# finsberg/fenicsx-beat

Hardware: AMD Instinct MI355X
Metric: node_updates_per_sec (higher is better)
Workload: dtype f64

## Files before the change

### fenicsx-beat_amd/beat/_engine.py

```python

from __future__ import annotations

import ctypes as C
import os
from dataclasses import dataclass
from typing import Any

import numpy as np

from . import _hip


@dataclass
class Slab:

    nz_global: int
    rank: int = 0
    world: int = 1
    weights: Any = None

    def __post_init__(self):
        if self.world > self.nz_global:
            raise ValueError(f"{self.world} ranks for only {self.nz_global} z-planes")
        if self.weights is not None and self.world > 1:
# ... 345 lines not shown
        if isinstance(order, str):
            if order != "auto":
                raise ValueError(f"guess order must be an integer 0..4 or 'auto', got {order!r}")
            order = -1
        self.flush_pending()
        _hip.check(self.lib.beat_pde_set_guess_order(self.handle, int(order)))
        self.guess_order = int(order)

    def set_single_reduction(self, on) -> None:
        _hip.check(self.lib.beat_pde_set_single_reduction(self.handle, -1 if on is None else int(bool(on))))

    def set_small(self, enable: bool) -> None:
        _hip.check(self.lib.beat_pde_set_small_grid_solve(self.handle, int(bool(enable))))

    def small_active(self) -> bool:
        return bool(self.lib.beat_pde_small_grid_solve_active(self.handle))

    RR_ROUTE_KEYS = ("available", "ry", "pd", "by_rows_mask", "nsegx", "nrb", "zc", "nchunks", "total_blocks", "guess_ry")

    def rr_route(self) -> dict:
        out = (C.c_int * len(self.RR_ROUTE_KEYS))()
        _hip.check(self.lib.beat_pde_rr_route(self.handle, out))
        return {k: int(v) for k, v in zip(self.RR_ROUTE_KEYS, out)}

    def guess_traffic(self) -> dict:
        out = (C.c_int * 4)()
        _hip.check(self.lib.beat_pde_guess_traffic(self.handle, out))
        return {"reads": int(out[0]), "writes": int(out[1]), "order": int(out[2]), "pending": bool(out[3])}

    def guess_reset(self) -> None:
        self.flush_pending()
        _hip.check(self.lib.beat_pde_guess_reset(self.handle))

    def flush_pending(self) -> None:
        if self.open_x is not None:
            self.solve_finish()
        if self.pending is not None:
            x, ring_base, _ = self.pending
            self.pending = None
            self.flushes = getattr(self, "flushes", 0) + 1
            _hip.check(self.lib.beat_pde_x_flush(self.handle, C.c_void_p(self.st_ptr_for_flush), x.ptr, self.ring[0].ptr,
                                                 self.fld, ring_base, 0))

    def flush_pending_events(self, field, maps, t0: float, t1: float) -> bool:
        if self.open_x is not None:
            self.solve_finish()
# ... 485 lines not shown
```

### fenicsx-beat_amd/beat/_hip.py

```python

from __future__ import annotations

import ctypes as C
import os
from pathlib import Path

_HERE = Path(__file__).resolve().parent
_LIB_PATH = Path(os.environ.get("BEAT_HIP_LIBRARY", _HERE / "lib" / "libbeat_hip.so"))

MODEL_SIMPLE_ODE = 0
MODEL_FHN_DEMO = 1
MODEL_FHN_README = 2
MODEL_TP06_GRL1 = 3
MODEL_TORORD_DYNCL_GRL1 = 4
MODEL_TORORD_LAND_GRL1 = 5
(MATH_EXP, MATH_EXP_INT, MATH_LOG, MATH_LOG_INT, MATH_RCP, MATH_RSQRT, MATH_TP06_RCP2, MATH_TP06_RCP3, MATH_TP06_RCP4,
 MATH_TORORD_RCP2, MATH_TORORD_RCP3, MATH_TORORD_RCP4, MATH_TP06_PHI_SMALL, MATH_TP06_PHI7, MATH_TORORD_PHI_SMALL,
 MATH_TORORD_PHI7, MATH_TP06_GRL1, MATH_TP06_ADVANCE, MATH_TP06_GATE, MATH_TORORD_ADVANCE, MATH_TORORD_GATE,
 MATH_TORORD_GATE_B) = range(22)
MATH_IN = (1, 1, 1, 1, 1, 1, 2, 3, 4, 2, 3, 4, 1, 1, 1, 1, 4, 4, 4, 4, 4, 4)
MATH_OUT = (1, 1, 1, 1, 1, 1, 2, 3, 4, 2, 3, 4, 1, 1, 1, 1, 1, 1, 1, 1, 1, 1)
MAX_STIM = 8
MAX_CLASSES = 32
MAX_LEADS = 16
# ... 80 lines not shown
    "beat_pde_set_timestep": (_int, [_vp, _dbl, _dbl, _dbl]),
    "beat_pde_apply": (_int, [_vp, _int, _vp, _vp]),
    "beat_pde_rhs": (_int, [_vp, _vp, C.POINTER(_vp), C.POINTER(_dbl), _int, _vp, _vp, _vp, _vp]),
    "beat_pde_cg_begin": (_int, [_vp, _vp, _dbl, _dbl, _int]),
    "beat_pde_spmv_dot": (_int, [_vp, _vp, _vp, _vp]),
    "beat_pde_spmv_dot_part": (_int, [_vp, _vp, _vp, _vp, _int]),
    "beat_pde_cg_update": (_int, [_vp, _vp, _vp, _vp, _vp, _vp]),
    "beat_pde_cg_next": (_int, [_vp, _vp, _vp, _vp]),
    "beat_pde_ring_size": (_int, []),
    "beat_pde_cg_update_r": (_int, [_vp, _vp, _vp, _vp, _int]),
    "beat_pde_cg_next_oop": (_int, [_vp, _vp, _vp, _vp, _vp]),
    "beat_pde_x_flush": (_int, [_vp, _vp, _vp, _vp, _i64, _int, _int]),
    "beat_pde_set_small_grid_solve": (_int, [_vp, _int]),
    "beat_pde_small_grid_solve_active": (_int, [_vp]),
    "beat_split_steps": (_int, [_vp, _int, _vp, _i64, _i64, _vp, _int, _int, _vp, _int, _vp, _vp, _vp, _vp, _int, _dbl, _dbl,
                                _int, _vp, _vp, _int, _vp, _vp]),
    "beat_split_steps_big": (_int, [_vp, _int, _vp, _i64, _i64, _vp, _int, _int, _vp, _vp, _int, _vp, _vp, _vp, _vp, _int, _dbl, _dbl, _int, _int,
                             C.POINTER(KspInfo), C.POINTER(_int), C.POINTER(C.c_float)]),
    "beat_pde_set_guess_order": (_int, [_vp, _int]),
    "beat_pde_set_single_reduction": (_int, [_vp, _int]),
    "beat_pde_fused_dist_pass": (_int, [_vp]),
    "beat_pde_tile_route": (_int, [_vp]),
    "beat_pde_rr_route": (_int, [_vp, C.POINTER(_int)]),
    "beat_pde_guess_reset": (_int, [_vp]),
    "beat_pde_guess_pending": (_int, [_vp]),
    "beat_pde_guess_history": (_int, [_vp, _vp, _vp, _vp]),
    "beat_pde_guess_traffic": (_int, [_vp, C.POINTER(_int)]),
    "beat_pde_set_preconditioner": (_int, [_vp, _int, _vp]),
    "beat_pde_pc_num_passes": (_int, [_vp]),
    "beat_pde_pc_pass": (_int, [_vp, _int, _vp, _vp, _vp, _vp, _vp]),
    "beat_pde_cg_first_z": (_int, [_vp, _vp, _vp, _vp]),
    "beat_pde_cg_next_z": (_int, [_vp, _vp, _vp, _vp]),
    "beat_pde_work_fields": (_int, [_vp]),
    "beat_pde_field_stride": (_i64, [_vp]),
    "beat_pde_solve": (
        _int,
        [_vp, _vp, C.POINTER(_vp), C.POINTER(_dbl), _int, _vp, _vp, _dbl, _dbl, _int, C.POINTER(KspInfo)],
    ),
    "beat_pde_solve_begin": (_int, [_vp, _vp, C.POINTER(_vp), C.POINTER(_dbl), _int, _vp, _vp, _dbl, _dbl, _int]),
    "beat_pde_solve_end": (_int, [_vp, C.POINTER(KspInfo), C.POINTER(_int)]),
    "beat_pde_solve_is_open": (_int, [_vp]),
    "beat_pde_solve_can_open": (_int, [_vp]),
    "beat_pde_solve_ex": (
        _int,
        [_vp, _vp, C.POINTER(_vp), C.POINTER(_dbl), _int, _vp, _vp, _dbl, _dbl, _int, _int, C.POINTER(KspInfo), C.POINTER(_int)],
    ),
# ... 93 lines not shown
```

### fenicsx-beat_amd/csrc/beat_pde_rr.hip

```cpp
#include "beat_pde_internal.h"

#include <algorithm>
#include <cmath>
#include <cstddef>
#include <cstdlib>

namespace {
using namespace beat_pde_detail;

constexpr int SEG = 62;

struct Coef {
  double c[15];
};

struct RGeom {
  int nx, ny, nz;
  int64_t plane;
  int ry;
  int nsegx, nrb, nchunks, zc;
  int total_waves, total_blocks;
  int z_lo_phys, z_hi_phys;
  int z_lo, z_hi;
  int part_off;
// ... 84 lines not shown
#define BEAT_RR_ALIGN_RHS 0
#endif
constexpr bool rr_aligned_mode(int mode) {
  return BEAT_RR_ALIGN == 1 && BEAT_RR_BUF != 0 && (mode == 0 || mode == 1 || mode == 3 || mode == 4 || (mode == 2 && BEAT_RR_ALIGN_RHS == 1));
}

__device__ __forceinline__ int axis_type3(int i, int n, int lo_phys, int hi_phys) {
  if (n == 1 && lo_phys && hi_phys) return 1;
  if (i == 0 && lo_phys) return 0;
  if (i == n - 1 && hi_phys) return 2;
  return 1;
}

__device__ __forceinline__ int xcd_block(int b, int total) {
  const int per = (total + 7) >> 3;
  return (b & 7) * per + (b >> 3);
}

#ifndef BEAT_RR_WAVES_RHS
#define BEAT_RR_WAVES_RHS 3
#endif
#ifndef BEAT_RR_WAVES_IT
#define BEAT_RR_WAVES_IT 1
#endif
template <int MODE, int RY, int PD, bool GUESS = false, bool PRED = false>
__global__ __launch_bounds__(BEAT_BLOCK, (GUESS && RY == 2 && PD == 1) ? BEAT_RR_WAVES_RHS : ((MODE == RR_PDOT || MODE == RR_RUPD) && PD == 1 ? BEAT_RR_WAVES_IT : 1)) void rr_kernel(RGeom g, RArgs a, const double* __restrict__ X,
                                                        const double* __restrict__ X2, double* __restrict__ Y,
                                                        double* __restrict__ Y2) {
  constexpr int NR = RY + 2;
  constexpr int NE = GUESS ? NR : 1;
  constexpr bool FORM = MODE == RR_PDOT || MODE == RR_UDOT || MODE == RR_PRUPD;
  constexpr bool OLD = MODE == RR_PDOT || MODE == RR_PRUPD;
  constexpr bool RAW = MODE == RR_UDOT || MODE == RR_PRUPD;
  constexpr int NW = RAW ? RY : 1;
  constexpr bool BUF = BEAT_RR_BUF == 1 || (BEAT_RR_BUF == 2 && (MODE != RR_RHS || BEAT_RR_ALIGN_RHS == 1));
  constexpr bool ALIGNED = rr_aligned_mode(MODE);
  static_assert(!ALIGNED || BUF, "aligned segments come with the raw-buffer loads");
  constexpr int SEGW = ALIGNED ? 64 : SEG;
  static_assert(!GUESS || MODE == RR_RHS, "the initial guess enters the right-hand side only");
  static_assert(!PRED || MODE == RR_PDOT, "the predicted-stop sums come with PDOT only");
  __shared__ double red[4];
  __shared__ double s_dinv[32];
  __shared__ double s_tab[27 * TABW];
  __shared__ double s_tab2[MODE == RR_RHS ? 27 * TABW : 1];
  __shared__ double s_taba[GUESS ? 27 * TABW : 1];
  __shared__ double s_rc[PRED ? 4 * 2 * RY * 64 : 1];
// ... 358 lines not shown
  if (MODE == RR_PDOT && !PRED) {
    const double s0 = beat_block_sum(acc0, red);
    if (threadIdx.x == 0) a.partials[g.part_off + blockIdx.x] = s0;
  } else if (MODE == RR_RUPD) {
    const double s0 = beat_block_sum(acc0, red);
    const double s1 = beat_block_sum(acc1, red);
    if (threadIdx.x == 0) {
      a.partials[g.part_off + blockIdx.x] = s0;
      a.partials[BEAT_MAX_PARTIALS + g.part_off + blockIdx.x] = s1;
    }
  } else if (MODE == RR_PRUPD) {
  } else {
    const double s0 = beat_block_sum(acc0, red);
    const double s1 = beat_block_sum(acc1, red);
    const double s2 = beat_block_sum(acc2, red);
    if (threadIdx.x == 0) {
      a.partials[g.part_off + blockIdx.x] = s0;
      a.partials[BEAT_MAX_PARTIALS + g.part_off + blockIdx.x] = s1;
      a.partials[2 * BEAT_MAX_PARTIALS + g.part_off + blockIdx.x] = s2;
    }
  }
}

__global__ void rr_next_kernel(double* st) {
  if (st[STOP] != 0.0) return;
  st[BETA] = st[RZN] / st[RZ];
  st[RZ] = st[RZN];
  st[RR] = st[RRN];
  st[ITERS] += 1.0;
  const double tr = st[RTOL] * st[RTOL] * st[BB];
  if (st[RR] <= st[TOL2]) {
    st[STOP] = 1.0;
    st[REASON] = st[RR] <= tr ? 2.0 : 3.0;
  } else if (st[ITERS] >= st[MAXIT]) {
    st[STOP] = 1.0;
    st[REASON] = -3.0;
  }
}

__global__ void rr_merged_next_kernel(double* st, double* alphas, int slot) {
  if (st[STOP] != 0.0) return;
  const double g = st[RZN], d = st[PQ], rr = st[RRN];
  st[RR] = rr;
  const double tr = st[RTOL] * st[RTOL] * st[BB];
  if (rr <= st[TOL2]) {
    st[STOP] = 1.0;
// ... 37 lines not shown
    const int v = e ? std::atoi(e) : 1;
    return (v >= 1 && v <= 3) ? v : 1;
  }();
  return pd;
}

int rr_guess_rows() {
  static const int rows = [] {
    const char* e = std::getenv("BEAT_RR_GUESS_RY");
    const int v = e ? std::atoi(e) : 2;
    return v == 4 ? 4 : 2;
  }();
  return rows;
}

int rr_by_rows_mask() {
  static const int mask = [] {
    const char* e = std::getenv("BEAT_RR_BY_ROWS");
    return e ? std::atoi(e) : 0;
  }();
  return mask;
}

RGeom make_geom(const beat_pde* pde, int z_lo, int z_hi, int part_off, int rows = 0, int mode = -1) {
  const Geom& f = pde->g;
  RGeom g{};
  const int64_t nodes = (int64_t)f.nx * f.ny * f.nz;
  const int RY = g.ry = rows ? rows : rr_rows(nodes);
  g.nx = f.nx;
  g.ny = f.ny;
  g.nz = f.nz;
  g.plane = f.plane;
  g.z_lo_phys = f.z_lo_phys;
  g.z_hi_phys = f.z_hi_phys;
  g.z_lo = z_lo;
  g.z_hi = z_hi;
  g.part_off = part_off;
  g.ghost_lo_tz = pde->ghost_lo_tz;
  g.ghost_hi_tz = pde->ghost_hi_tz;
  const int segw = (mode >= 0 && rr_aligned_mode(mode)) ? 64 : SEG;
  g.nsegx = (f.nx + segw - 1) / segw;
  g.nrb = (f.ny + RY - 1) / RY;
  const int nzr = std::max(0, z_hi - z_lo);
  g.nrg = (mode >= 0 && ((rr_by_rows_mask() >> mode) & 1)) ? (g.nrb + 3) / 4 : 0;
  const int64_t per_layer = g.nrg > 0 ? (int64_t)g.nsegx * g.nrg : ((int64_t)g.nsegx * g.nrb + 3) / 4;
  const int target = rr_target_blocks(nodes);
  int nchunks = (int)std::max<int64_t>(1, (target + per_layer - 1) / per_layer);
  nchunks = std::max(1, std::min(nchunks, nzr));
  g.zc = std::max(1, (nzr + nchunks - 1) / nchunks);
  g.nchunks = (nzr + g.zc - 1) / g.zc;
  while ((int64_t)g.nsegx * g.nrb * g.nchunks > (int64_t)2 * BEAT_MAX_PARTIALS && g.nchunks > 1) {
    g.zc *= 2;
    g.nchunks = (nzr + g.zc - 1) / g.zc;
  }
  g.total_waves = g.nsegx * g.nrb * g.nchunks;
  g.total_blocks = (g.total_waves + 3) / 4;
  if (g.nrg > 0) {
    g.total_blocks = g.nsegx * g.nrg * g.nchunks;
    g.total_waves = g.total_blocks * 4;
  }
  return g;
}

// ... 14 lines not shown
  a.dinv = pde->d_dinv();
  a.ci = interior_row(pde->h_A);
  a.dinv_i = pde->h_dinv[13];
  a.partials = pde->ctx->d_partials;
  a.st = dev_st;
  return a;
}

template <int MODE, bool GUESS = false, bool PRED = false>
void launch_rr(const beat_pde* pde, const RGeom& g, const RArgs& a) {
  if (g.total_blocks <= 0) return;
  const dim3 grid((unsigned)grid_blocks(g)), block(BEAT_BLOCK);
  hipStream_t s = pde->ctx->stream;
#define BEAT_RR_LAUNCH(RYV, PDV) \
  BEAT_KERNEL((rr_kernel<MODE, RYV, PDV, GUESS, PRED>), grid, block, 0, s, g, a, a.x, GUESS ? a.e : a.x2, a.y, a.y2)
  const int pd = rr_prefetch();
  if (g.ry == 2) {
    if (pd == 2) BEAT_RR_LAUNCH(2, 2); else if (pd == 3) BEAT_RR_LAUNCH(2, 3); else BEAT_RR_LAUNCH(2, 1);
  } else {
    if (pd == 2) BEAT_RR_LAUNCH(4, 2); else if (pd == 3) BEAT_RR_LAUNCH(4, 3); else BEAT_RR_LAUNCH(4, 1);
  }
#undef BEAT_RR_LAUNCH
}
}

bool beat_rr_available(const beat_pde* pde) {
  if (pde->var || pde->pc_ncoef != 1) return false;
  if (const char* e = std::getenv("BEAT_RR")) {
    if (e[0] == '0') return false;
  }
  const RGeom g = make_geom(pde);
  const RGeom gb = make_geom(pde, 0, 1, 0);
  return (int64_t)grid_blocks(g) + 2 * grid_blocks(gb) <= BEAT_MAX_PARTIALS;
}

extern "C" int beat_pde_rr_route(const beat_pde* pde, int* host_out) {
  BEAT_REQUIRE(pde != nullptr && host_out != nullptr, "null argument");
  const RGeom g = make_geom(pde, 0, pde->g.nz, 0, 0, RR_PDOT);
  host_out[0] = beat_rr_available(pde) ? 1 : 0;
  host_out[1] = g.ry;
  host_out[2] = rr_prefetch();
  host_out[3] = rr_by_rows_mask();
  host_out[4] = g.nsegx;
  host_out[5] = g.nrb;
  host_out[6] = g.zc;
  host_out[7] = g.nchunks;
  host_out[8] = g.total_blocks;
  host_out[9] = rr_guess_rows();
  return BEAT_OK;
}

int beat_rr_rhs(beat_pde* pde, const double* dev_v_prev, const double* const* host_dev_stim_w, const double* host_stim_amp,
                int n_stim, double* dev_x, double* dev_r, double* dev_st, int part, const PcgStart* start) {
  BEAT_REQUIRE(start == nullptr || part < 0, "only a right-hand side in one part starts the solve");
  const GuessTerms& gt = pde->guess.cur;
  const bool guess = gt.d != nullptr && gt.use_e;
  const int rows = guess ? rr_guess_rows() : 0;
  RArgs a{};
  a.x = dev_v_prev;
  a.y = dev_r;
  a.y2 = (dev_x == dev_v_prev) ? nullptr : dev_x;
  a.tab = pde->d_tab(2);
  a.tab2 = pde->d_tab(3);
  a.dinv = pde->d_dinv();
  a.ci = interior_row(pde->h_mass);
  a.ci2 = interior_row(pde->h_stiff);
  a.dinv_i = pde->h_dinv[13];
  a.cm = pde->C_m;
  a.omt_dt = (1.0 - pde->theta) * pde->dt;
  a.dt = pde->dt;
  beat_fill_stimuli(a, host_dev_stim_w, host_stim_amp, n_stim);
// ... 2 lines not shown
  if (guess) {
    a.tab = pde->d_tab(1);
    a.ci = interior_row(pde->h_B);
    a.e = gt.e;
    a.taba = pde->d_tab(0);
    a.cia = interior_row(pde->h_A);
  }
  auto launch = [&](int z_lo, int z_hi, int part_off) {
    const RGeom g = make_geom(pde, z_lo, z_hi, part_off, rows, RR_RHS);
    if (guess)
      launch_rr<RR_RHS, true>(pde, g, a);
    else
      launch_rr<RR_RHS>(pde, g, a);
    return blocks_written(g);
  };
  int count = 0;
  if (int rc = beat_launch_parts(pde, PASS_RR_RHS, part, launch, &count)) return rc;
  return part == 0 ? BEAT_OK : beat_pde_launch_reduce(pde, count, 3, dev_st, nullptr, ScalarStep::begin(dev_st, start));
}

double beat_rr_predict_bound(const beat_pde* pde) {
  const Geom& f = pde->g;
  int depth = 0;
  auto chain = [&](const RGeom& g) {
    const int per_thread = (grid_blocks(g) + BEAT_BLOCK - 1) / BEAT_BLOCK;
    depth = std::max(depth, g.zc * g.ry + 8 + per_thread + 8);
  };
  chain(make_geom(pde, 0, f.nz, 0, 0, RR_RHS));
  chain(make_geom(pde, 0, f.nz, 0, 2, RR_RHS));
  chain(make_geom(pde, 0, f.nz, 0, 4, RR_RHS));
  chain(make_geom(pde, 0, f.nz, 0, 0, RR_PDOT));
  chain(make_geom(pde, 0, f.nz, 0, 0, RR_RUPD));
  return 4.0 * (2.0 * depth + 8.0) * std::ldexp(1.0, -53);
}

int beat_rr_pdot_part(beat_pde* pde, double* dev_st, const double* dev_r, const double* dev_p_old, double* dev_p_new,
                      int part, int slot) {
  const Geom& f = pde->g;
  const bool pred = slot >= 0 && pde->predict_stop && f.z_lo_phys && f.z_hi_phys;
  if (pred && pde->predict_c <= 0.0) pde->predict_c = beat_rr_predict_bound(pde);
  RArgs a = rr_operator_args(pde, dev_st);
  a.x = dev_r;
  a.x2 = dev_p_old;
  a.y = dev_p_new;
  auto launch = [&](int z_lo, int z_hi, int part_off) {
    const RGeom g = make_geom(pde, z_lo, z_hi, part_off, 0, RR_PDOT);
    if (pred)
      launch_rr<RR_PDOT, false, true>(pde, g, a);
    else
      launch_rr<RR_PDOT>(pde, g, a);
    return blocks_written(g);
  };
  int count = 0;
  if (int rc = beat_launch_parts(pde, PASS_RR_PDOT, part, launch, &count)) return rc;
  if (part == 0) return BEAT_OK;
  if (pred) {
    static_assert(RQ == PQS + 1 && QQ == PQS + 2, "the three sums are reduced into one run of slots");
    ScalarStep predict{ScalarStep::PREDICT, dev_st};
    predict.alpha_slot = pde->d_alphas + slot;
    predict.bound_c = pde->predict_c;
    return beat_pde_launch_reduce(pde, count, 3, dev_st + PQS, dev_st, predict);
  }
  return beat_pde_launch_reduce(pde, count, 1, dev_st + PQ, dev_st);
}

int beat_rr_pdot(beat_pde* pde, double* dev_st, const double* dev_r, const double* dev_p_old, double* dev_p_new, int slot) {
  if (int rc = beat_rr_pdot_part(pde, dev_st, dev_r, dev_p_old, dev_p_new, 0, slot)) return rc;
  return beat_rr_pdot_part(pde, dev_st, dev_r, dev_p_old, dev_p_new, 1, slot);
}

int beat_rr_rupd(beat_pde* pde, double* dev_st, const double* dev_r, double* dev_r_new, const double* dev_p, int slot,
                 bool roll) {
  const RGeom g = make_geom(pde, 0, pde->g.nz, 0, 0, RR_RUPD);
  RArgs a = rr_operator_args(pde, dev_st);
  a.x = dev_p;
  a.x2 = dev_r;
  a.y = dev_r_new;
  a.alphas = pde->d_alphas;
  a.slot = slot;
  launch_rr<RR_RUPD>(pde, g, a);
  BEAT_LAUNCH_CHECK();
  return beat_pde_launch_reduce(pde, grid_blocks(g), 2, dev_st + RZN, dev_st, ScalarStep::after_update(dev_st, roll));
}

int beat_rr_udot_part(beat_pde* pde, double* dev_st, const double* dev_r, int part) {
  static_assert(RZN == PQ + 1 && RRN == PQ + 2, "the three sums travel as one all-reduce of dev_st[PQ..RRN]");
  RArgs a = rr_operator_args(pde, dev_st);
  a.x = dev_r;
  a.x2 = dev_r;
  auto launch = [&](int z_lo, int z_hi, int part_off) {
    const RGeom g = make_geom(pde, z_lo, z_hi, part_off, 0, RR_UDOT);
    launch_rr<RR_UDOT>(pde, g, a);
    return blocks_written(g);
  };
  int count = 0;
  if (int rc = beat_launch_parts(pde, PASS_RR_UDOT, part, launch, &count)) return rc;
  return part == 0 ? BEAT_OK : beat_pde_launch_reduce(pde, count, 3, dev_st + PQ, dev_st);
}

int beat_rr_merged_next(beat_pde* pde, double* dev_st, int slot) {
  BEAT_KERNEL(rr_merged_next_kernel, dim3(1), dim3(1), 0, pde->ctx->stream, dev_st, pde->d_alphas, slot);
  BEAT_LAUNCH_CHECK();
  return BEAT_OK;
// ... 21 lines not shown
```

### fenicsx-beat_amd/csrc/beat_probe.hip

```cpp
#include "beat_common.h"
#include "beat_math_probe.h"

namespace {

typedef double v2d __attribute__((ext_vector_type(2)));
typedef int v4i __attribute__((ext_vector_type(4)));

template <int POL>
__device__ __forceinline__ v2d ld16(const v2d* base, int64_t i) {
  if constexpr (POL & 4) {
    const int64_t blk = i >> 26;
    const __amdgpu_buffer_rsrc_t r = __builtin_amdgcn_make_buffer_rsrc((void*)(base + (blk << 26)), 0, 0x7ffffff0, 0x00020000);
    const v4i v = __builtin_amdgcn_raw_buffer_load_b128(r, (int)((i - (blk << 26)) * 16), 0, (POL & 1) ? 2 : 0);
    return __builtin_bit_cast(v2d, v);
  } else if constexpr (POL & 1) {
    return __builtin_nontemporal_load(base + i);
  } else {
    return base[i];
  }
}
template <int POL>
__device__ __forceinline__ void st16(v2d* base, int64_t i, v2d v) {
  if constexpr (POL & 4) {
    const int64_t blk = i >> 26;
// ... 121 lines not shown
    for (int r = 0; r < NR; ++r) nxt[r] = src[(int64_t)zn * plane + off[r]];
    double hnxt = 0.0;
    if (halo) {
      const __amdgpu_buffer_rsrc_t rs = __builtin_amdgcn_make_buffer_rsrc((void*)(src + (int64_t)zn * plane), 0, (int)(plane * 8), 0x00020000);
      typedef int v2i __attribute__((ext_vector_type(2)));
      const v2i hv = __builtin_amdgcn_raw_buffer_load_b64(rs, (int)hoff, 0, 0);
      hnxt = __hiloint2double(hv.y, hv.x);
    }
    if (out) {
#pragma unroll
      for (int j = 0; j < RY; ++j) {
        const int gy = rb * RY + j;
        if (gy < ny) dst[(int64_t)z * plane + (int64_t)gy * nx + gx] = cur[j] + cur[j + 1] + cur[j + 2] + (lane == 0 ? hcur : 0.0);
      }
    }
    hsum += hcur;
#pragma unroll
    for (int r = 0; r < NR; ++r) cur[r] = nxt[r];
    hcur = hnxt;
  }
  if (hsum == 1.2345e300) dst[0] = hsum;
}

int launch_march(beat_ctx* ctx, double* dev, int64_t n, int nx, int ry, int segw, int shift, int blocks, int halo) {
  BEAT_REQUIRE(nx >= 64 && (segw == 62 || segw == 64) && (shift == 0 || shift == -1) && (ry == 2 || ry == 4), "bad march probe arguments");
  const int64_t per_field = n / 2;
  const int nz = (int)(per_field / ((int64_t)nx * nx));
  BEAT_REQUIRE(nz >= 1 && (int64_t)nz * nx * nx == per_field, "the buffer holds two fields of nx x nx x nz doubles");
  const int nseg = (nx + segw - 1) / segw, nrb = (nx + ry - 1) / ry;
  const int64_t per_layer = ((int64_t)nseg * nrb + 3) / 4;
  int nchunks = (int)std::max<int64_t>(1, ((blocks > 0 ? blocks : 4096) + per_layer - 1) / per_layer);
  nchunks = std::min(nchunks, nz);
  const int zc = (nz + nchunks - 1) / nchunks;
  nchunks = (nz + zc - 1) / zc;
  const int total_waves = nseg * nrb * nchunks;
  const unsigned grid = (unsigned)((total_waves + 3) / 4);
  if (ry == 4)
    BEAT_KERNEL((march_kernel<4>), dim3(grid), dim3(BEAT_BLOCK), 0, ctx->stream, (const double*)dev, dev + per_field, nx, nx, nz, segw, shift, zc, total_waves, halo);
  else
    BEAT_KERNEL((march_kernel<2>), dim3(grid), dim3(BEAT_BLOCK), 0, ctx->stream, (const double*)dev, dev + per_field, nx, nx, nz, segw, shift, zc, total_waves, halo);
  BEAT_LAUNCH_CHECK();
  return BEAT_OK;
}

__global__ __launch_bounds__(BEAT_BLOCK) void math_probe_kernel(int fn, const double* __restrict__ in, int64_t ld, double* __restrict__ out,
                                                                int64_t n) {
  __shared__ double etab[BEAT_EXP_TAB], etabi[BEAT_EXP_TAB];
  __shared__ LogEntry ltab[128];
  static_assert(BEAT_EXP_TAB == BEAT_BLOCK, "one table entry per thread");
  etab[threadIdx.x] = beat_exp_tab_entry<false>(kExp2Tab[threadIdx.x], (int)threadIdx.x);
  etabi[threadIdx.x] = beat_exp_tab_entry<true>(kExp2Tab[threadIdx.x], (int)threadIdx.x);
  if (threadIdx.x < 128) ltab[threadIdx.x] = kLogTab[threadIdx.x];
  __syncthreads();
  FastMath fm{etab, ltab};
  FastMathT<true> fmi{etabi, ltab};
  beat_fm_pin(fm);
  beat_fm_pin(fmi);
  const int64_t i = (int64_t)blockIdx.x * BEAT_BLOCK + threadIdx.x;
  if (i >= n) return;
  double a[4], o[4];
// ... 52 lines not shown
```

### include/beat_hip.h

```cpp
#ifndef BEAT_HIP_H
#define BEAT_HIP_H

#include <stddef.h>
#include <stdint.h>

#ifdef __cplusplus
extern "C" {
#endif

#define BEAT_OK 0
#define BEAT_EINVAL -1
#define BEAT_EHIP -2
#define BEAT_ENOTCONV -3
#define BEAT_ENOMEM -4

#define BEAT_ABI_VERSION 1

#define BEAT_MODEL_SIMPLE_ODE 0
#define BEAT_MODEL_FHN_DEMO 1
#define BEAT_MODEL_FHN_README 2
#define BEAT_MODEL_TP06_GRL1 3

#define BEAT_MODEL_TORORD_DYNCL_GRL1 4
#define BEAT_MODEL_TORORD_LAND_GRL1 5
// ... 99 lines not shown
int beat_pde_cg_next(beat_pde* pde, double* dev_st, const double* dev_r, double* dev_p);

int beat_pde_ring_size(void);
int beat_pde_cg_update_r(beat_pde* pde, double* dev_st, double* dev_r, const double* dev_q, int slot);
int beat_pde_cg_next_oop(beat_pde* pde, double* dev_st, const double* dev_r, const double* dev_p_cur,
                         double* dev_p_next);
int beat_pde_x_flush(beat_pde* pde, const double* dev_st, double* dev_x, const double* dev_ring0,
                     int64_t field_stride, int ring_base, int only_if_full);

int beat_pde_set_preconditioner(beat_pde* pde, int ncoef, const double* host_coef);
int beat_pde_pc_num_passes(beat_pde* pde);
int beat_pde_pc_pass(beat_pde* pde, int j, const double* dev_r, double* dev_z, double* dev_q,
                     double* dev_st, double* dev_red);
int beat_pde_cg_first_z(beat_pde* pde, double* dev_st, const double* dev_z, double* dev_p);
int beat_pde_cg_next_z(beat_pde* pde, double* dev_st, const double* dev_z, double* dev_p);

int beat_pde_work_fields(beat_pde* pde);
int64_t beat_pde_field_stride(const beat_pde* pde);
int beat_pde_set_guess_order(beat_pde* pde, int order);
int beat_pde_set_single_reduction(beat_pde* pde, int on);
int beat_pde_fused_dist_pass(const beat_pde* pde);
int beat_pde_tile_route(const beat_pde* pde);
int beat_pde_rr_route(const beat_pde* pde, int* host_out);
int beat_pde_guess_reset(beat_pde* pde);
int beat_pde_guess_pending(const beat_pde* pde);
int beat_pde_guess_history(const beat_pde* pde, double** dev_d, double** dev_e, int* count);
int beat_pde_guess_traffic(const beat_pde* pde, int* host_out);

int beat_pde_set_small_grid_solve(beat_pde* pde, int enable);
int beat_pde_small_grid_solve_active(const beat_pde* pde);

#define BEAT_MAX_BATCH 1024
int beat_split_steps(beat_ctx* ctx, int model_id, double* dev_states, int64_t n, int64_t ld,
                     const double* host_params, int num_params, int v_index, beat_pde* pde, int n_steps,
                     const double* host_t0, const double* host_dt, const double* const* host_dev_stim_w, const double* host_stim_amp, int n_stim,
                     double rtol, double atol, int max_it, const int64_t* host_probe_idx, const double* host_probe_w,
                     int n_probe, double* dev_probe_out, beat_ksp_info* host_info);
int beat_split_steps_big(beat_ctx* ctx, int model_id, double* dev_states, int64_t n, int64_t ld, const double* host_params,
                         int num_params, int v_index, beat_pde* pde, double* dev_work, int n_steps, const double* host_t0,
                         const double* host_dt, const double* const* host_dev_stim_w, const double* host_stim_amp, int n_stim,
                         double rtol, double atol, int max_it, int pending_in, beat_ksp_info* host_info, int* host_pending,
                         float* host_ode_ms);

int beat_pde_solve_begin(beat_pde* pde, const double* dev_v_prev, const double* const* host_dev_stim_w,
                         const double* host_stim_amp, int n_stim, double* dev_x, double* dev_work, double rtol, double atol, int max_it);
int beat_pde_solve_end(beat_pde* pde, beat_ksp_info* info, int* host_pending);
// ... 92 lines not shown
```

Baseline: 11.29 billion.

## Process two x-nodes per lane in the CG stencil pdot and residual-update kernels

Adds an rr2_kernel variant in which each lane handles two adjacent x nodes using 128-bit buffer loads and stores, with segments widened to 128 nodes. It is used by default for the PDOT and RUPD iteration passes when nx is even and the aligned prefetch route is active. The aim is to halve the number of load/store instructions and give each lane more independent arithmetic, at the cost of higher register pressure and a 16-byte alignment requirement on the vectors. A matching march probe kernel and a query for the element count are also added.

```diff
diff --git a/fenicsx-beat_amd/beat/_engine.py b/fenicsx-beat_amd/beat/_engine.py
--- a/fenicsx-beat_amd/beat/_engine.py
+++ b/fenicsx-beat_amd/beat/_engine.py
@@ -391,6 +391,11 @@
         out = (C.c_int * len(self.RR_ROUTE_KEYS))()
         _hip.check(self.lib.beat_pde_rr_route(self.handle, out))
         return {k: int(v) for k, v in zip(self.RR_ROUTE_KEYS, out)}
+
+    def rr_elems(self) -> int:
+        out = (C.c_int * 1)()
+        _hip.check(self.lib.beat_pde_rr_elems(self.handle, out))
+        return int(out[0])
 
     def guess_traffic(self) -> dict:
         out = (C.c_int * 4)()
diff --git a/fenicsx-beat_amd/beat/_hip.py b/fenicsx-beat_amd/beat/_hip.py
--- a/fenicsx-beat_amd/beat/_hip.py
+++ b/fenicsx-beat_amd/beat/_hip.py
@@ -126,6 +126,7 @@
     "beat_pde_fused_dist_pass": (_int, [_vp]),
     "beat_pde_tile_route": (_int, [_vp]),
     "beat_pde_rr_route": (_int, [_vp, C.POINTER(_int)]),
+    "beat_pde_rr_elems": (_int, [_vp, C.POINTER(_int)]),
     "beat_pde_guess_reset": (_int, [_vp]),
     "beat_pde_guess_pending": (_int, [_vp]),
     "beat_pde_guess_history": (_int, [_vp, _vp, _vp, _vp]),
diff --git a/fenicsx-beat_amd/csrc/beat_pde_rr.hip b/fenicsx-beat_amd/csrc/beat_pde_rr.hip
--- a/fenicsx-beat_amd/csrc/beat_pde_rr.hip
+++ b/fenicsx-beat_amd/csrc/beat_pde_rr.hip
@@ -130,6 +130,9 @@
 #endif
 #ifndef BEAT_RR_WAVES_IT
 #define BEAT_RR_WAVES_IT 1
+#endif
+#ifndef BEAT_RR_ELEMS_DEFAULT
+#define BEAT_RR_ELEMS_DEFAULT 2
 #endif
 template <int MODE, int RY, int PD, bool GUESS = false, bool PRED = false>
 __global__ __launch_bounds__(BEAT_BLOCK, (GUESS && RY == 2 && PD == 1) ? BEAT_RR_WAVES_RHS : ((MODE == RR_PDOT || MODE == RR_RUPD) && PD == 1 ? BEAT_RR_WAVES_IT : 1)) void rr_kernel(RGeom g, RArgs a, const double* __restrict__ X,
@@ -534,6 +537,252 @@
   }
 }
 
+typedef double rr_v2d __attribute__((ext_vector_type(2)));
+typedef int rr_v4i __attribute__((ext_vector_type(4)));
+constexpr int SEG2 = 128;
+__device__ __forceinline__ rr_v2d rr_buf_load2(const double* base, unsigned bytes, unsigned off) {
+  const __amdgpu_buffer_rsrc_t r = __builtin_amdgcn_make_buffer_rsrc((void*)base, 0, (int)bytes, 0x00020000);
+  return __builtin_bit_cast(rr_v2d, __builtin_amdgcn_raw_buffer_load_b128(r, (int)off, 0, (BEAT_RR_NT & 1) ? 2 : 0));
+}
+__device__ __forceinline__ void rr_store2(double* p, rr_v2d v) {
+#if BEAT_RR_NT & 2
+  __builtin_nontemporal_store(v, (rr_v2d*)p);
+#else
+  *(rr_v2d*)p = v;
+#endif
+}
+
+template <int MODE, int RY, bool PRED = false>
+__global__ __launch_bounds__(BEAT_BLOCK, BEAT_RR_WAVES_IT) void rr2_kernel(RGeom g, RArgs a, const double* __restrict__ X,
+                                                                             const double* __restrict__ X2, double* __restrict__ Y) {
+  static_assert(MODE == RR_PDOT || MODE == RR_RUPD, "two nodes per lane: the iteration's two passes only");
+  static_assert(!PRED || MODE == RR_PDOT, "the predicted-stop sums come with PDOT only");
+  static_assert(rr_aligned_mode(MODE), "the aligned raw-buffer form");
+  constexpr int NR = RY + 2;
+  constexpr bool FORM = MODE == RR_PDOT;
+  __shared__ double red[4];
+  __shared__ double s_dinv[32];
+  __shared__ double s_tab[27 * TABW];
+  __shared__ double s_rc[PRED ? 4 * 2 * RY * 128 : 1];
+  __shared__ double s_acc[PRED ? 4 * 2 * 64 : 1];
+  if (a.st[STOP] != 0.0) return;
+  if (PRED) s_acc[(threadIdx.x >> 6) * 128 + (threadIdx.x & 63)] = s_acc[(threadIdx.x >> 6) * 128 + 64 + (threadIdx.x & 63)] = 0.0;
+  for (int i = threadIdx.x; i < 27 * TABW; i += BEAT_BLOCK) s_tab[i] = a.tab[i];
+  if (threadIdx.x < 27) s_dinv[threadIdx.x] = a.dinv[threadIdx.x];
+  __syncthreads();
+  const int lane = threadIdx.x & 63;
+  const int blk = xcd_block(blockIdx.x, g.total_blocks);
+  const int w = blk * 4 + (threadIdx.x >> 6);
+  int seg = w % g.nsegx;
+  int rb = (w / g.nsegx) % g.nrb;
+  int chunk = w / (g.nsegx * g.nrb);
+  bool wave_ok = blk < g.total_blocks && w < g.total_waves;
+  if (g.nrg > 0) {
+    seg = blk % g.nsegx;
+    rb = ((blk / g.nsegx) % g.nrg) * 4 + (int)(threadIdx.x >> 6);
+    chunk = blk / (g.nsegx * g.nrg);
+    wave_ok = blk < g.total_blocks && rb < g.nrb;
+  }
+  const int gx = seg * SEG2 + 2 * lane;
+  const int y0 = rb * RY - 1;
+  const int zb = g.z_lo + chunk * g.zc;
+  const int ze = wave_ok ? min(zb + g.zc, g.z_hi) : zb;
+  const bool x_in = wave_ok && gx < g.nx;
+  const int tx0 = axis_type3(gx, g.nx, 1, 1), tx1 = axis_type3(min(gx + 1, g.nx - 1), g.nx, 1, 1);
+  bool row_in[NR];
+  int ty3[NR];
+  unsigned off[NR];
+#pragma unroll
+  for (int r = 0; r < NR; ++r) {
+    const int gy = y0 + r;
+    row_in[r] = x_in && gy >= 0 && gy < g.ny;
+    ty3[r] = 3 * axis_type3(gy, g.ny, 1, 1);
+    off[r] = row_in[r] ? (unsigned)(gy * g.nx + gx) * 8u : RR_OOB;
+  }
+  const unsigned pbytes = (unsigned)(g.plane * 8);
+  unsigned hoff = RR_OOB;
+  int htxy;
+  {
+    const int hr = lane < 8 ? lane : lane - 8;
+    const int hx = lane < 8 ? seg * SEG2 - 1 : seg * SEG2 + SEG2;
+    const int hy = y0 + hr;
+    const bool hv = wave_ok && (lane < NR || (lane >= 8 && lane < 8 + NR)) && hx >= 0 && hx < g.nx && hy >= 0 && hy < g.ny;
+    hoff = hv ? (unsigned)(hy * g.nx + hx) * 8u : RR_OOB;
+    htxy = axis_type3(min(max(hx, 0), g.nx - 1), g.nx, 1, 1) + 3 * axis_type3(min(max(hy, 0), g.ny - 1), g.ny, 1, 1);
+  }
+  double beta = 0.0, alpha = 0.0;
+  if (FORM) beta = a.st[BETA];
+  if (MODE == RR_RUPD) {
+    alpha = a.st[RZ] / a.st[PQ];
+    if (blockIdx.x == 0 && threadIdx.x == 0) a.alphas[a.slot] = alpha;
+  }
+  const bool have_old = beta != 0.0;
+
+  double acc0 = 0.0, acc1 = 0.0, acc2 = 0.0;
+  const rr_v2d zero2 = {0.0, 0.0};
+  rr_v2d Cm[NR], C0[NR], Cp[NR], ra[NR], rb2[NR], rvn[RY];
+  double Hm = 0.0, H0 = 0.0, Hp = 0.0, rha = 0.0, rhb = 0.0;
+#pragma unroll
+  for (int r = 0; r < NR; ++r) Cm[r] = C0[r] = Cp[r] = ra[r] = rb2[r] = zero2;
+#pragma unroll
+  for (int j = 0; j < RY; ++j) rvn[j] = zero2;
+  for (int z = zb - 3; z < ze; ++z) {
+    const int k = z + 1;
+    if (k >= zb - 1 && k <= ze) {
+      const int tz9 = 9 * (k < 0 ? g.ghost_lo_tz : k >= g.nz ? g.ghost_hi_tz : axis_type3(k, g.nz, g.z_lo_phys, g.z_hi_phys));
+      const bool own_plane = (k >= zb && k < ze) || (k == -1 && zb == 0 && !g.z_lo_phys) || (k == g.nz && ze == g.nz && !g.z_hi_phys);
+#pragma unroll
+      for (int r = 0; r < NR; ++r) {
+        rr_v2d c = ra[r];
+        if (FORM) {
+          const double d0 = s_dinv[tx0 + ty3[r] + tz9], d1 = s_dinv[tx1 + ty3[r] + tz9];
+          c.x = have_old ? fma(beta, rb2[r].x, d0 * ra[r].x) : d0 * ra[r].x;
+          c.y = have_old ? fma(beta, rb2[r].y, d1 * ra[r].y) : d1 * ra[r].y;
+        }
+        Cp[r] = c;
+        if (FORM) {
+          if (own_plane && r >= 1 && r <= RY && row_in[r]) rr_store2(&Y[(int64_t)k * g.plane + (int64_t)(y0 + r) * g.nx + gx], c);
+        }
+        if (PRED && r >= 1 && r <= RY) {
+          double* sr = &s_rc[((((threadIdx.x >> 6) * 2 + (k & 1)) * RY) + r - 1) * 128 + lane];
+          sr[0] = ra[r].x;
+          sr[64] = ra[r].y;
+        }
+      }
+      double hc = rha;
+      if (FORM) {
+        const double di = s_dinv[htxy + tz9];
+        hc = have_old ? fma(beta, rhb, di * rha) : di * rha;
+      }
+      Hp = hc;
+    }
+    rr_v2d rv[RY];
+    if (MODE == RR_RUPD) {
+#pragma unroll
+      for (int j = 0; j < RY; ++j) rv[j] = rvn[j];
+      if (z + 1 >= zb && z + 1 < ze) {
+        const double* __restrict__ br = X2 + (int64_t)(z + 1) * g.plane;
+#pragma unroll
+        for (int j = 0; j < RY; ++j) rvn[j] = rr_buf_load2(br, pbytes, off[j + 1]);
+      }
+    }
+    {
+      const int kf = k + 1;
+      if (kf >= zb - 1 && kf <= ze) {
+        const int cz = min(max(kf, -1), g.nz);
+        const double* __restrict__ bx = X + (int64_t)cz * g.plane;
+        const double* __restrict__ bx2 = (FORM && have_old) ? X2 + (int64_t)cz * g.plane : bx;
+        const unsigned pb = ((kf >= 0 || !g.z_lo_phys) && (kf < g.nz || !g.z_hi_phys)) ? pbytes : 0u;
+#pragma unroll
+        for (int r = 0; r < NR; ++r) {
+          ra[r] = rr_buf_load2(bx, pb, off[r]);
+          if (FORM) rb2[r] = rr_buf_load2(bx2, pb, off[r]);
+        }
+        rha = rr_buf_load(bx, pb, hoff);
+        if (FORM) rhb = rr_buf_load(bx2, pb, hoff);
+      }
+    }
+    if (z >= zb) {
+      double L0[NR], R0[NR], Rp[NR], Lm[NR];
+#pragma unroll
+      for (int r = 0; r < NR - 1; ++r) {
+        L0[r] = from_left_h(C0[r].y, H0, r);
+        Lm[r] = from_left_h(Cm[r].y, Hm, r);
+      }
+#pragma unroll
+      for (int r = 1; r < NR; ++r) {
+        R0[r] = from_right_h(C0[r].x, H0, 8 + r);
+        Rp[r] = from_right_h(Cp[r].x, Hp, 8 + r);
+      }
+      const int tz = axis_type3(z, g.nz, g.z_lo_phys, g.z_hi_phys);
+#pragma unroll
+      for (int j = 0; j < RY; ++j) {
+        const int r = j + 1;
+        if (row_in[r]) {
+          const int64_t gi = (int64_t)z * g.plane + (int64_t)(y0 + r) * g.nx + gx;
+          rr_v2d res = zero2;
+#pragma unroll
+          for (int e = 0; e < 2; ++e) {
+            double v[15];
+            v[0] = e ? C0[r].y : C0[r].x;
+            v[1] = e ? R0[r] : C0[r].y;
+            v[2] = e ? C0[r].x : L0[r];
+            v[3] = e ? C0[r + 1].y : C0[r + 1].x;
+            v[4] = e ? C0[r - 1].y : C0[r - 1].x;
+            v[5] = e ? Cp[r].y : Cp[r].x;
+            v[6] = e ? Cm[r].y : Cm[r].x;
+            v[7] = e ? R0[r + 1] : C0[r + 1].y;
+            v[8] = e ? C0[r - 1].x : L0[r - 1];
+            v[9] = e ? Cp[r + 1].y : Cp[r + 1].x;
+            v[10] = e ? Cm[r - 1].y : Cm[r - 1].x;
+            v[11] = e ? Rp[r] : Cp[r].y;
+            v[12] = e ? Cm[r].x : Lm[r];
+            v[13] = e ? Rp[r + 1] : Cp[r + 1].y;
+            v[14] = e ? Cm[r - 1].x : Lm[r - 1];
+            const int type = (e ? tx1 : tx0) + ty3[r] + 9 * tz;
+            double s = 0.0;
+#pragma unroll
+            for (int k2 = 0; k2 < 15; ++k2) s = fma(a.ci.c[k2], v[k2], s);
+            double di = s_dinv[13];
+            if (type != 13) {
+              s = 0.0;
+#pragma unroll
+              for (int k2 = 0; k2 < 15; ++k2) s = fma(s_tab[type * TABW + k2], v[k2], s);
+              di = s_dinv[type];
+            }
+            if (MODE == RR_PDOT) {
+              acc0 = fma(v[0], s, acc0);
+              if (PRED) {
+                double* sa = &s_acc[(threadIdx.x >> 6) * 128 + lane];
+                sa[0] = fma(s_rc[((((threadIdx.x >> 6) * 2 + (z & 1)) * RY) + j) * 128 + e * 64 + lane], s, sa[0]);
+                sa[64] = fma(s, s, sa[64]);
+              }
+            } else {
+              const double ri = fma(-alpha, s, e ? rv[j].y : rv[j].x);
+              if (e) res.y = ri; else res.x = ri;
+              acc0 = fma(ri * di, ri, acc0);
+              acc1 = fma(ri, ri, acc1);
+            }
+          }
+          if (MODE == RR_RUPD) rr_store2(&Y[gi], res);
+        }
+      }
+    }
+#pragma unroll
+    for (int r = 0; r < NR; ++r) {
+      Cm[r] = C0[r];
+      C0[r] = Cp[r];
+    }
+    Hm = H0;
+    H0 = Hp;
+  }
+
+  if (PRED) {
+    acc1 = s_acc[(threadIdx.x >> 6) * 128 + (threadIdx.x & 63)];
+    acc2 = s_acc[(threadIdx.x >> 6) * 128 + 64 + (threadIdx.x & 63)];
+  }
+  if (MODE == RR_PDOT && !PRED) {
+    const double s0 = beat_block_sum(acc0, red);
+    if (threadIdx.x == 0) a.partials[g.part_off + blockIdx.x] = s0;
+  } else if (MODE == RR_RUPD) {
+    const double s0 = beat_block_sum(acc0, red);
+    const double s1 = beat_block_sum(acc1, red);
+    if (threadIdx.x == 0) {
+      a.partials[g.part_off + blockIdx.x] = s0;
+      a.partials[BEAT_MAX_PARTIALS + g.part_off + blockIdx.x] = s1;
+    }
+  } else {
+    const double s0 = beat_block_sum(acc0, red);
+    const double s1 = beat_block_sum(acc1, red);
+    const double s2 = beat_block_sum(acc2, red);
+    if (threadIdx.x == 0) {
+      a.partials[g.part_off + blockIdx.x] = s0;
+      a.partials[BEAT_MAX_PARTIALS + g.part_off + blockIdx.x] = s1;
+      a.partials[2 * BEAT_MAX_PARTIALS + g.part_off + blockIdx.x] = s2;
+    }
+  }
+}
+
 __global__ void rr_next_kernel(double* st) {
   if (st[STOP] != 0.0) return;
   st[BETA] = st[RZN] / st[RZ];
@@ -617,7 +866,19 @@
   return mask;
 }
 
-RGeom make_geom(const beat_pde* pde, int z_lo, int z_hi, int part_off, int rows = 0, int mode = -1) {
+int rr_elems_wanted() {
+  static const int elems = [] {
+    const char* e = std::getenv("BEAT_RR_ELEMS");
+    const int v = e ? std::atoi(e) : BEAT_RR_ELEMS_DEFAULT;
+    return v == 2 ? 2 : 1;
+  }();
+  return elems;
+}
+int rr_elems(const beat_pde* pde) {
+  return (rr_elems_wanted() == 2 && rr_aligned_mode(RR_PDOT) && rr_aligned_mode(RR_RUPD) && (pde->g.nx & 1) == 0 && rr_prefetch() == 1) ? 2 : 1;
+}
+
+RGeom make_geom(const beat_pde* pde, int z_lo, int z_hi, int part_off, int rows = 0, int mode = -1, int segw = 0) {
   const Geom& f = pde->g;
   RGeom g{};
   const int64_t nodes = (int64_t)f.nx * f.ny * f.nz;
@@ -633,7 +894,10 @@
   g.part_off = part_off;
   g.ghost_lo_tz = pde->ghost_lo_tz;
   g.ghost_hi_tz = pde->ghost_hi_tz;
-  const int segw = (mode >= 0 && rr_aligned_mode(mode)) ? 64 : SEG;
+  if (segw == 0) {
+    segw = (mode >= 0 && rr_aligned_mode(mode)) ? 64 : SEG;
+    if ((mode == RR_PDOT || mode == RR_RUPD) && rr_elems(pde) == 2) segw = SEG2;
+  }
   g.nsegx = (f.nx + segw - 1) / segw;
   g.nrb = (f.ny + RY - 1) / RY;
   const int nzr = std::max(0, z_hi - z_lo);
@@ -694,6 +958,20 @@
   }
 #undef BEAT_RR_LAUNCH
 }
+
+inline bool rr_pairs_aligned(const RArgs& a) {
+  return (((uintptr_t)a.x | (uintptr_t)a.x2 | (uintptr_t)a.y) & 15) == 0;
+}
+template <int MODE, bool PRED = false>
+void launch_rr2(const beat_pde* pde, const RGeom& g, const RArgs& a) {
+  if (g.total_blocks <= 0) return;
+  const dim3 grid((unsigned)grid_blocks(g)), block(BEAT_BLOCK);
+  hipStream_t s = pde->ctx->stream;
+  if (g.ry == 2)
+    BEAT_KERNEL((rr2_kernel<MODE, 2, PRED>), grid, block, 0, s, g, a, a.x, a.x2, a.y);
+  else
+    BEAT_KERNEL((rr2_kernel<MODE, 4, PRED>), grid, block, 0, s, g, a, a.x, a.x2, a.y);
+}
 }
 
 bool beat_rr_available(const beat_pde* pde) {
@@ -719,6 +997,12 @@
   host_out[7] = g.nchunks;
   host_out[8] = g.total_blocks;
   host_out[9] = rr_guess_rows();
+  return BEAT_OK;
+}
+
+extern "C" int beat_pde_rr_elems(const beat_pde* pde, int* host_out) {
+  BEAT_REQUIRE(pde != nullptr && host_out != nullptr, "null argument");
+  host_out[0] = rr_elems(pde);
   return BEAT_OK;
 }
 
@@ -767,15 +1051,15 @@
 double beat_rr_predict_bound(const beat_pde* pde) {
   const Geom& f = pde->g;
   int depth = 0;
-  auto chain = [&](const RGeom& g) {
+  auto chain = [&](const RGeom& g, int elems = 1) {
     const int per_thread = (grid_blocks(g) + BEAT_BLOCK - 1) / BEAT_BLOCK;
-    depth = std::max(depth, g.zc * g.ry + 8 + per_thread + 8);
+    depth = std::max(depth, g.zc * g.ry * elems + 8 + per_thread + 8);
   };
   chain(make_geom(pde, 0, f.nz, 0, 0, RR_RHS));
   chain(make_geom(pde, 0, f.nz, 0, 2, RR_RHS));
   chain(make_geom(pde, 0, f.nz, 0, 4, RR_RHS));
-  chain(make_geom(pde, 0, f.nz, 0, 0, RR_PDOT));
-  chain(make_geom(pde, 0, f.nz, 0, 0, RR_RUPD));
+  chain(make_geom(pde, 0, f.nz, 0, 0, RR_PDOT), rr_elems(pde));
+  chain(make_geom(pde, 0, f.nz, 0, 0, RR_RUPD), rr_elems(pde));
   return 4.0 * (2.0 * depth + 8.0) * std::ldexp(1.0, -53);
 }
 
@@ -788,9 +1072,15 @@
   a.x = dev_r;
   a.x2 = dev_p_old;
   a.y = dev_p_new;
+  BEAT_REQUIRE(rr_elems(pde) == 1 || rr_pairs_aligned(a), "two nodes per lane: r, p_old and p_new must be 16-byte aligned");
   auto launch = [&](int z_lo, int z_hi, int part_off) {
     const RGeom g = make_geom(pde, z_lo, z_hi, part_off, 0, RR_PDOT);
-    if (pred)
+    if (rr_elems(pde) == 2) {
+      if (pred)
+        launch_rr2<RR_PDOT, true>(pde, g, a);
+      else
+        launch_rr2<RR_PDOT>(pde, g, a);
+    } else if (pred)
       launch_rr<RR_PDOT, false, true>(pde, g, a);
     else
       launch_rr<RR_PDOT>(pde, g, a);
@@ -823,7 +1113,12 @@
   a.y = dev_r_new;
   a.alphas = pde->d_alphas;
   a.slot = slot;
-  launch_rr<RR_RUPD>(pde, g, a);
+  if (rr_elems(pde) == 2) {
+    BEAT_REQUIRE(rr_pairs_aligned(a), "two nodes per lane: r, r_new and p must be 16-byte aligned");
+    launch_rr2<RR_RUPD>(pde, g, a);
+  } else {
+    launch_rr<RR_RUPD>(pde, g, a);
+  }
   BEAT_LAUNCH_CHECK();
   return beat_pde_launch_reduce(pde, grid_blocks(g), 2, dev_st + RZN, dev_st, ScalarStep::after_update(dev_st, roll));
 }
diff --git a/fenicsx-beat_amd/csrc/beat_probe.hip b/fenicsx-beat_amd/csrc/beat_probe.hip
--- a/fenicsx-beat_amd/csrc/beat_probe.hip
+++ b/fenicsx-beat_amd/csrc/beat_probe.hip
@@ -167,8 +167,73 @@
   if (hsum == 1.2345e300) dst[0] = hsum;
 }
 
+template <int RY>
+__global__ __launch_bounds__(BEAT_BLOCK) void march2_kernel(const double* __restrict__ src, double* __restrict__ dst, int nx, int ny, int nz,
+                                                            int zc, int total_waves, int halo) {
+  constexpr int NR = RY + 2;
+  constexpr int SEGW = 128;
+  constexpr unsigned OOB = 0x80000000u;
+  const int lane = threadIdx.x & 63;
+  const int w = blockIdx.x * 4 + (threadIdx.x >> 6);
+  if (w >= total_waves) return;
+  const int nseg = (nx + SEGW - 1) / SEGW, nrb = (ny + RY - 1) / RY;
+  const int seg = w % nseg, rb = (w / nseg) % nrb, chunk = w / (nseg * nrb);
+  const int gx = seg * SEGW + 2 * lane;
+  const bool out = gx < nx;
+  const int64_t plane = (int64_t)nx * ny;
+  const unsigned pbytes = (unsigned)(plane * 8);
+  unsigned off[NR];
+#pragma unroll
+  for (int r = 0; r < NR; ++r) {
+    const int gy = rb * RY - 1 + r;
+    off[r] = (out && gy >= 0 && gy < ny) ? (unsigned)(gy * nx + gx) * 8u : OOB;
+  }
+  const int hr = lane < 8 ? lane : lane - 8;
+  const bool hl = halo && ((lane < NR) || (lane >= 8 && lane < 8 + NR));
+  const int hx = lane < 8 ? seg * SEGW - 1 : seg * SEGW + SEGW;
+  const int hy = rb * RY - 1 + hr;
+  const unsigned hoff = (hl && hx >= 0 && hx < nx && hy >= 0 && hy < ny) ? (unsigned)(hy * nx + hx) * 8u : OOB;
+  const int zb = chunk * zc, ze = min(zb + zc, nz);
+  v2d cur[NR], nxt[NR];
+  {
+    const __amdgpu_buffer_rsrc_t rs = __builtin_amdgcn_make_buffer_rsrc((void*)(src + (int64_t)zb * plane), 0, (int)pbytes, 0x00020000);
+#pragma unroll
+    for (int r = 0; r < NR; ++r) cur[r] = __builtin_bit_cast(v2d, __builtin_amdgcn_raw_buffer_load_b128(rs, (int)off[r], 0, 0));
+  }
+  double hcur = 0.0, hsum = 0.0;
+  for (int z = zb; z < ze; ++z) {
+    const int zn = min(z + 1, nz - 1);
+    const __amdgpu_buffer_rsrc_t rs = __builtin_amdgcn_make_buffer_rsrc((void*)(src + (int64_t)zn * plane), 0, (int)pbytes, 0x00020000);
+#pragma unroll
+    for (int r = 0; r < NR; ++r) nxt[r] = __builtin_bit_cast(v2d, __builtin_amdgcn_raw_buffer_load_b128(rs, (int)off[r], 0, 0));
+    double hnxt = 0.0;
+    if (halo) {
+      typedef int v2i __attribute__((ext_vector_type(2)));
+      const v2i hv = __builtin_amdgcn_raw_buffer_load_b64(rs, (int)hoff, 0, 0);
+      hnxt = __hiloint2double(hv.y, hv.x);
+    }
+    if (out) {
+#pragma unroll
+      for (int j = 0; j < RY; ++j) {
+        const int gy = rb * RY + j;
+        if (gy < ny) {
+          v2d s = cur[j] + cur[j + 1] + cur[j + 2];
+          s.x += lane == 0 ? hcur : 0.0;
+          __builtin_nontemporal_store(s, (v2d*)(dst + (int64_t)z * plane + (int64_t)gy * nx + gx));
+        }
+      }
+    }
+    hsum += hcur;
+#pragma unroll
+    for (int r = 0; r < NR; ++r) cur[r] = nxt[r];
+    hcur = hnxt;
+  }
+  if (hsum == 1.2345e300) dst[0] = hsum;
+}
+
 int launch_march(beat_ctx* ctx, double* dev, int64_t n, int nx, int ry, int segw, int shift, int blocks, int halo) {
-  BEAT_REQUIRE(nx >= 64 && (segw == 62 || segw == 64) && (shift == 0 || shift == -1) && (ry == 2 || ry == 4), "bad march probe arguments");
+  BEAT_REQUIRE(nx >= 64 && (segw == 62 || segw == 64 || segw == 128) && (shift == 0 || shift == -1) && (ry == 2 || ry == 4), "bad march probe arguments");
+  BEAT_REQUIRE(segw != 128 || (shift == 0 && (nx & 1) == 0 && (int64_t)nx * nx * 8 < ((int64_t)1 << 31)), "two nodes per lane: aligned segments, an even nx and a plane below 2 GiB");
   const int64_t per_field = n / 2;
   const int nz = (int)(per_field / ((int64_t)nx * nx));
   BEAT_REQUIRE(nz >= 1 && (int64_t)nz * nx * nx == per_field, "the buffer holds two fields of nx x nx x nz doubles");
@@ -180,7 +245,11 @@
   nchunks = (nz + zc - 1) / zc;
   const int total_waves = nseg * nrb * nchunks;
   const unsigned grid = (unsigned)((total_waves + 3) / 4);
-  if (ry == 4)
+  if (segw == 128 && ry == 4)
+    BEAT_KERNEL((march2_kernel<4>), dim3(grid), dim3(BEAT_BLOCK), 0, ctx->stream, (const double*)dev, dev + per_field, nx, nx, nz, zc, total_waves, halo);
+  else if (segw == 128)
+    BEAT_KERNEL((march2_kernel<2>), dim3(grid), dim3(BEAT_BLOCK), 0, ctx->stream, (const double*)dev, dev + per_field, nx, nx, nz, zc, total_waves, halo);
+  else if (ry == 4)
     BEAT_KERNEL((march_kernel<4>), dim3(grid), dim3(BEAT_BLOCK), 0, ctx->stream, (const double*)dev, dev + per_field, nx, nx, nz, segw, shift, zc, total_waves, halo);
   else
     BEAT_KERNEL((march_kernel<2>), dim3(grid), dim3(BEAT_BLOCK), 0, ctx->stream, (const double*)dev, dev + per_field, nx, nx, nz, segw, shift, zc, total_waves, halo);
diff --git a/include/beat_hip.h b/include/beat_hip.h
--- a/include/beat_hip.h
+++ b/include/beat_hip.h
@@ -145,6 +145,7 @@
 int beat_pde_fused_dist_pass(const beat_pde* pde);
 int beat_pde_tile_route(const beat_pde* pde);
 int beat_pde_rr_route(const beat_pde* pde, int* host_out);
+int beat_pde_rr_elems(const beat_pde* pde, int* host_out);
 int beat_pde_guess_reset(beat_pde* pde);
 int beat_pde_guess_pending(const beat_pde* pde);
 int beat_pde_guess_history(const beat_pde* pde, double** dev_d, double** dev_e, int* count);
```

New measurement: 11.46 billion, median of 6. 1.01x the previous value.
